# noahchalifour/rnnt-speech-recognition

Hardware: AMD Instinct MI355X
Metric: rnnt_loss_grad_lattice_cells_per_sec (higher is better)
Workload: dtype f32

## Files before the change

rnnt-speech-recognition_amd/csrc/rnnt_cell.h:

```cpp
#pragma once
#include "rnnt_common.h"

namespace rnnt {

__device__ __forceinline__ int length_T(const LossParams &p, const int b) { return min(max(p.input_lengths[b], 1), p.T); }
__device__ __forceinline__ int length_U(const LossParams &p, const int b) { return min(max(p.label_lengths[b] + 1, 1), p.U); }
__device__ __forceinline__ bool lengths_invalid(const LossParams &p, const int b) {
    const int t = p.input_lengths[b], l = p.label_lengths[b];
    return t < 1 || t > p.T || l < 0 || l > p.U - 1;
}

struct Cell {
    int b, t, u, Tb, Ub;
    bool valid;
};

__device__ __forceinline__ Cell decode(const LossParams &p, uint32_t c) {
    Cell r;
    r.b = r.t = r.u = r.Tb = r.Ub = 0;
    r.valid = false;
    if (c < p.cells) {
        const uint32_t row = fdiv(c, p.divU);
        r.u = (int)(c - row * (uint32_t)p.U);
        const uint32_t b = fdiv(row, p.divT);
        r.t = (int)(row - b * (uint32_t)p.T);
        r.b = (int)b;
        r.Tb = length_T(p, (int)b);
        r.Ub = length_U(p, (int)b);
        r.valid = (r.t < r.Tb) && (r.u < r.Ub);
    }
    return r;
}

__device__ __forceinline__ int clamp_label(int lab, int V) { return min(max(lab, 0), V - 1); }

template <bool SC1>
__device__ __forceinline__ float ld_f32(const float *q) {
    return SC1 ? __hip_atomic_load(q, __ATOMIC_RELAXED, __HIP_MEMORY_SCOPE_AGENT) : *q;
}
template <bool SC1>
__device__ __forceinline__ double ld_f64(const double *q) {
    return SC1 ? __hip_atomic_load(q, __ATOMIC_RELAXED, __HIP_MEMORY_SCOPE_AGENT) : *q;
}
__device__ __forceinline__ void st_f32_wt(float *q, float v) {
    __hip_atomic_store(q, v, __ATOMIC_RELAXED, __HIP_MEMORY_SCOPE_AGENT);
}
__device__ __forceinline__ void st_f64_wt(double *q, double v) {
    __hip_atomic_store(q, v, __ATOMIC_RELAXED, __HIP_MEMORY_SCOPE_AGENT);
}
struct CellGrad {
    float c0;
    float nl;
    float cb;
    float cl;
    bool has_blank_corr, has_label;
    int lab;
    float scale;
    float bscale, lscale;
};

template <bool SC1 = false>
__device__ __forceinline__ CellGrad cell_grad_from(const LossParams &p, const Cell &cl, uint32_t c, const float a, const float bt,
                                                   const float b_t1, const float b_u1) {
    CellGrad g;
    const int n = cl.t + cl.u;
    const int kc = n / kRebase, kc1 = (n + 1) / kRebase;
    const int g0 = (int)fdiv((uint32_t)cl.u, p.divOG), g1 = (int)fdiv((uint32_t)cl.u + 1u, p.divOG);
    const size_t ob = (size_t)cl.b * p.NC * p.NG;
    const double oa = (double)ld_f32<SC1>(p.offA + ob + (size_t)kc * p.NG + g0);
    const double ll2 = ld_f64<SC1>(p.ll + 2 * cl.b);
    const double da = (double)a + (oa - ll2);
    g.scale = p.cost_scale ? p.cost_scale[cl.b] : 1.0f;
    g.nl = -p.lse[c] * kLog2e;
    g.c0 = (float)(da + ((double)bt + (double)ld_f32<SC1>(p.offB + ob + (size_t)kc * p.NG + g0))) + g.nl;
    g.has_blank_corr = true;
    if (cl.t < cl.Tb - 1)
        g.cb = (float)(da + ((double)b_t1 + (double)ld_f32<SC1>(p.offB + ob + (size_t)kc1 * p.NG + g0)));
    else if (cl.u == cl.Ub - 1)
        g.cb = (float)da;
    else {
        g.cb = 0.f;
        g.has_blank_corr = false;
    }
    g.has_label = cl.u < cl.Ub - 1;
    g.lab = 0;
    g.cl = 0.f;
    if (g.has_label) {
        g.lab = clamp_label(p.labels[(size_t)cl.b * (p.U - 1) + cl.u], p.V);
        g.cl = (float)(da + ((double)b_u1 + (double)ld_f32<SC1>(p.offB + ob + (size_t)kc1 * p.NG + g1)));
    }
    return g;
}

__device__ __forceinline__ void fastemit_log(CellGrad &g, const float xl, const float lambda) {
    g.bscale = g.lscale = g.scale;
    if (g.has_label) {
        const float r = __builtin_amdgcn_exp2f(fminf((fmaf(xl, kLog2e, g.nl) + g.cl) - (g.c0 - g.nl), 0.f));
        g.lscale = fmaf(lambda, g.scale, g.scale);
        g.scale = fmaf(lambda * r, g.scale, g.scale);
    }
}

// ... 13 lines not shown
```

rnnt-speech-recognition_amd/csrc/rnnt_common.h:

```cpp
#pragma once
#include <hip/hip_runtime.h>
#include <stdint.h>

#include <type_traits>

namespace rnnt {

constexpr float kNeg = -1.0e30f;
constexpr float kNegTest = -1.0e29f;
constexpr float kLog2e = 1.4426950408889634f;
constexpr float kLn2 = 0.6931471805599453f;
constexpr int kRebase = 8;

struct FastDiv {
    uint32_t d, m, s;
};
inline FastDiv make_fastdiv(uint32_t d) {
    FastDiv f;
    f.d = d;
    uint32_t s = 0;
    while ((1ull << s) < d) ++s;
    f.s = s;
    f.m = (uint32_t)((((1ull << s) - d) << 32) / d) + 1u;
    return f;
}
__device__ __forceinline__ uint32_t fdiv(uint32_t n, const FastDiv f) {
    return (__umulhi(n, f.m) + n) >> f.s;
}

struct TileGeom {
    int TT, UU, tiles_t, tiles_u, cpr;
    FastDiv div_tu, div_tt, divUU, div_cpr, divTT;
};

struct LossParams {
    const float *acts;
    float *grads;
    const int *labels;
    const int *label_lengths;
    const int *input_lengths;
    const float *cost_scale;
    float *costs;
    float *lse;
    float *W;
    float *A;
    float *Bt;
    float *offA;
    float *offB;
    double *ll;
    int *EA;
    int *EB;
    float *lik;
    int *flags;
    int NCl;
    float2 *pstat;
    int *lshift;
    int *bar;
    int nPstat;
    int pstatStride;
    int B, T, U, V, blank;
    int b0, nb;
    int visit_all;
    int precise;
    int N, Nr, Up, NC, NG;
    uint32_t cells;
    FastDiv divU, divT, divV, divOG;
    TileGeom tile;
    float fe_lambda;
};

struct WsLayout {
    size_t lse, W, A, Bt, offA, offB, ll, EA, EB, lik, flags, pstat, lshift, bar, total;
    int NCl, nPstat;
    int N, Nr, Up, NC, NG, OG;
};

inline size_t align_up(size_t x, size_t a) { return (x + a - 1) / a * a; }

constexpr int kMaxU = 8192;
inline int sweep_K(int U) {
    const int k = (U + 63) / 64;
    const int avail[] = {1, 2, 3, 4, 6, 8, 12, 16};
    for (int a : avail)
        if (k <= a) return a;
    return 0;
}
template <int K, int G>
struct SweepRing {
    static constexpr size_t kChunk = (size_t)G * 2 * 64 * K * sizeof(float);
    static constexpr int NB = (4 * kChunk + 16 <= 128 * 1024) ? 4 : 3;
    static constexpr size_t kBytes = NB * kChunk + 16;
    static_assert(kBytes <= 160 * 1024, "chunk ring exceeds the LDS");
};
template <typename F>
inline hipError_t sweep_dispatch(int U, F &&f) {
    using std::integral_constant;
    switch (sweep_K(U)) {
        case 1: return f(integral_constant<int, 1>(), integral_constant<int, 16>());
        case 2: return f(integral_constant<int, 2>(), integral_constant<int, 16>());
        case 3: return f(integral_constant<int, 3>(), integral_constant<int, 16>());
        case 4: return f(integral_constant<int, 4>(), integral_constant<int, 16>());
        case 6: return f(integral_constant<int, 6>(), integral_constant<int, 8>());
        case 8: return f(integral_constant<int, 8>(), integral_constant<int, 8>());
        case 12: return f(integral_constant<int, 12>(), integral_constant<int, 4>());
        case 16: return f(integral_constant<int, 16>(), integral_constant<int, 4>());
        default: return hipErrorInvalidValue;
    }
}
constexpr int kFillByte = 0xF1;

inline WsLayout make_layout(int T, int U, int B) {
    WsLayout w;
    w.N = T + U - 1;
    w.Nr = (int)align_up((size_t)w.N, 16);
    w.Up = sweep_K(U) ? 64 * sweep_K(U) : (int)align_up((size_t)U, 64);
    w.NC = w.Nr / kRebase + 1;
    w.OG = sweep_K(U) ? sweep_K(U) : 64;
    w.NG = w.Up / w.OG;
    size_t off = 0;
    auto take = [&](size_t bytes) {
        size_t o = off;
        off = align_up(off + bytes, 256);
// ... 26 lines not shown
    TileGeom g;
    const int nu = (U + 31) / 32;
    g.UU = (U + nu - 1) / nu;
    g.TT = 256 / g.UU;
    if (g.TT > T) g.TT = T;
    g.tiles_u = (U + g.UU - 1) / g.UU;
    g.tiles_t = (T + g.TT - 1) / g.TT;
    g.cpr = g.UU * V / 4;
    g.div_tu = make_fastdiv((uint32_t)g.tiles_u);
    g.div_tt = make_fastdiv((uint32_t)g.tiles_t);
    g.divUU = make_fastdiv((uint32_t)g.UU);
    g.divTT = make_fastdiv((uint32_t)(g.TT > 0 ? g.TT : 1));
    g.div_cpr = make_fastdiv((uint32_t)(g.cpr > 0 ? g.cpr : 1));
    return g;
}

inline bool fill_loss_params(LossParams &p, const float *acts, float *grads, const int *labels, const int *label_lengths,
                             const int *input_lengths, const float *cost_scale, int V, int B, float *costs, void *workspace,
                             int maxT, int maxU, int blank) {
    const long long cells = (long long)B * maxT * maxU;
    if (cells <= 0 || cells >= (1ll << 31)) return false;
    if (((uintptr_t)workspace & 255) != 0) return false;
    const WsLayout w = make_layout(maxT, maxU, B);
    char *ws = (char *)workspace;
    p.acts = acts;
    p.grads = grads;
    p.labels = labels;
    p.label_lengths = label_lengths;
    p.input_lengths = input_lengths;
    p.cost_scale = cost_scale;
    p.costs = costs;
    p.lse = (float *)(ws + w.lse);
    p.W = (float *)(ws + w.W);
    p.A = (float *)(ws + w.A);
    p.Bt = (float *)(ws + w.Bt);
    p.offA = (float *)(ws + w.offA);
    p.offB = (float *)(ws + w.offB);
    p.ll = (double *)(ws + w.ll);
    p.EA = (int *)(ws + w.EA);
    p.EB = (int *)(ws + w.EB);
    p.lik = (float *)(ws + w.lik);
    p.flags = (int *)(ws + w.flags);
    p.NCl = w.NCl;
    p.pstat = (float2 *)(ws + w.pstat);
    p.lshift = (int *)(ws + w.lshift);
    p.bar = (int *)(ws + w.bar);
    p.nPstat = w.nPstat;
    p.pstatStride = 4;
    p.B = B, p.T = maxT, p.U = maxU, p.V = V, p.blank = blank;
    p.b0 = 0, p.nb = B;
    p.precise = 0;
    p.visit_all = 0;
    p.fe_lambda = 0.f;
    p.tile = make_tile(maxT, maxU, V);
    p.N = w.N, p.Nr = w.Nr, p.Up = w.Up, p.NC = w.NC, p.NG = w.NG;
    p.cells = (uint32_t)cells;
    p.divU = make_fastdiv((uint32_t)maxU);
    p.divT = make_fastdiv((uint32_t)maxT);
    p.divV = make_fastdiv((uint32_t)V);
    p.divOG = make_fastdiv((uint32_t)w.OG);
    return true;
}

constexpr float kExpTabLimit = 43.0f;
constexpr float kExpTab2Log2e = 2.8853900817779268f;
#ifdef __HIPCC__
__device__ __forceinline__ float exp_tab(float x) { return __builtin_amdgcn_exp2f(x * kExpTab2Log2e); }
__device__ __forceinline__ bool exp_tab_out_of_range(float x) { return !(fabsf(x) <= kExpTabLimit); }
#endif

constexpr int kHookBlocks = 1024;
struct JointHooks {
    int prep_mode;
    int prefilled;
    unsigned *dmax_enc;
    unsigned *dmax_pred;
};

#ifdef __HIPCC__
__device__ __forceinline__ void lds_dma16(const void *global, void *lds) {
    __builtin_amdgcn_global_load_lds((__attribute__((address_space(1))) const void *)global, (__attribute__((address_space(3))) void *)lds, 16, 0, 0);
}
#endif

inline int device_cu_count() {
    int dev = 0, n = 0;
    if (hipGetDevice(&dev) != hipSuccess) return 256;
    if (hipDeviceGetAttribute(&n, hipDeviceAttributeMultiprocessorCount, dev) != hipSuccess || n <= 0) return 256;
    return n;
}
template <typename Kernel>
inline hipError_t set_lds(Kernel kernel, size_t bytes) {
    if (bytes <= 64 * 1024) return hipSuccess;
    return hipFuncSetAttribute((const void *)kernel, hipFuncAttributeMaxDynamicSharedMemorySize, (int)bytes);
}

hipError_t launch_fill(void *dst, int byte, size_t bytes, hipStream_t s);
hipError_t launch_fill2(void *dst0, int byte0, size_t bytes0, void *dst1, int byte1, size_t bytes1, hipStream_t s);

bool tile_path_ok(const LossParams &p, bool grad);
hipError_t launch_lsm(const LossParams &p, hipStream_t s);
hipError_t launch_sweeps(const LossParams &p, hipStream_t s);
hipError_t launch_grad(const LossParams &p, hipStream_t s);
bool lin_path_ok(const LossParams &p);
hipError_t launch_lsm_lin(const LossParams &p, hipStream_t s);
hipError_t launch_sweeps_lin(const LossParams &p, hipStream_t s);
hipError_t launch_grad_lin(const LossParams &p, hipStream_t s);
hipError_t launch_redo_lin(const LossParams &p, bool force, hipStream_t s);

}
```

rnnt-speech-recognition_amd/csrc/rnnt_entrypoint.hip:

```cpp
#include "../../include/rnnt.h"
#include "rnnt_common.h"
#include "rnnt_lin.h"
#include "rnnt_align.h"
#include "rnnt_decode_host.h"

using namespace rnnt;

namespace rnnt {
hipError_t joint_workspace_bytes(int T, int U, int B, int J, int V, int joint_dtype, size_t *bytes);
hipError_t joint_f16_backward_rows(void *workspace, int T, int U, int B, int J, int V, int rows[2], hipStream_t s);
hipError_t joint_backward_rows(void *workspace, int T, int U, int B, int J, int V, int rows[2], hipStream_t s);
hipError_t launch_joint_loss(const float *enc_proj, const float *pred_proj, const float *W2, const float *b2,
                             const int *labels, const int *label_lengths, const int *input_lengths,
                             const float *cost_scale, int J, int V, int B, int T, int U, int blank, float *costs,
                             float *d_enc_proj, float *d_pred_proj, float *dW2, float *db2, int joint_dtype,
                             int phases, void *workspace, hipStream_t s, const JointHooks *hooks, float fe_lambda);
hipError_t joint_aux_pointers(void *workspace, int T, int U, int B, int J, int V, float **expE, float **expP, float **tflag);
hipError_t launch_joint_prefill(void *workspace, int T, int U, int B, int J, int V, hipStream_t s);
bool joint_dtype_supported(int joint_dtype, int J, int V);
bool dense_supported(int H, int J);
hipError_t dense_workspace_bytes(int B, int T, int U, int H, int J, size_t base, size_t *bytes);
void dense_proj_pointers(void *workspace, int B, int T, int U, int H, int J, size_t base, float **enc_proj, float **pred_proj,
                         float **d_enc_proj, float **d_pred_proj);
void dense_hook_pointers(void *workspace, int B, int T, int U, int H, int J, size_t base, unsigned **dmax_enc, unsigned **dmax_pred);
// ... 8 lines not shown
                                   int B, int T, int U, float *logits, void *workspace, hipStream_t s);
bool prednet_layout_ok(const rnntPrednetBlock *blocks, int L, int E, int V, int Jp, int R, size_t *bytes);
hipError_t launch_prednet_begin(const float *emb, const rnntPrednetBlock *blocks, int L, int E, int V, const float *W1, int Jp, int R,
                                float *out, void *workspace, hipStream_t s);
hipError_t launch_prednet_step(const int *emitted, const int *parents, float *out, const rnntPrednetBlock *blocks, int L, int E,
                               int V, int Jp, int R, void *workspace, hipStream_t s);
hipError_t launch_prednet_reset(const int *reset, float *out, const rnntPrednetBlock *blocks, int L, int E, int V, int Jp, int R,
                                void *workspace, hipStream_t s);
bool encoder_layout_ok(const rnntPrednetBlock *blocks, int L, int F, float bn_eps, int ridx, int f, int R, int Tmax, size_t *bytes);
hipError_t launch_encoder_begin(const rnntPrednetBlock *blocks, int L, int F, const float *bn_mean, const float *bn_var,
                                const float *bn_weight, const float *bn_bias, float bn_eps, int ridx, int f, int R, int Tmax,
                                void *workspace, hipStream_t s);
hipError_t launch_encoder_run(const float *x, int T, float *out, const rnntPrednetBlock *blocks, int L, int F, float bn_eps, int ridx,
                              int f, int R, int Tmax, void *workspace, hipStream_t s);
hipError_t launch_encoder_run_rows(const float *x, int T, const int *row_frames, const int *reset, float *out,
                                   const rnntPrednetBlock *blocks, int L, int F, float bn_eps, int ridx, int f, int R, int Tmax,
                                   void *workspace, hipStream_t s);
bool lstm_train_layout_ok(int R, int T, int H, int P, bool proj, size_t *bytes);
hipError_t launch_lstm_train_fwd(float *gates, const float *W_hh, const float *W_hr, float *y, float *c, float *h, int R, int T, int H,
                                 int P, void *workspace, hipStream_t s);
hipError_t launch_lstm_train_bwd(float *gates, const float *c, const float *dy, const float *W_hh, const float *W_hr, float *dr, int R,
                                 int T, int H, int P, void *workspace, hipStream_t s);
bool frontend_layout_ok(int K, int S, int L, int step, int M, int stack, int rm, size_t *bytes, int *max_rows);
hipError_t launch_frontend_begin(const float *window, const float *mel_weights, int K, int S, int L, int step, int M, int stack,
                                 int rm, void *workspace, hipStream_t s);
hipError_t launch_frontend_feed(const float *audio, int cs, const int *samples, const int *reset, const int *final_, int norm,
                                float *rows, int *counts, int K, int S, int L, int step, int M, int stack, int rm, void *workspace,
                                hipStream_t s);
}

extern "C" {

int get_warprnnt_version(void) { return 1; }

const char *rnntGetStatusString(rnntStatus_t status) {
    switch (status) {
        case RNNT_STATUS_SUCCESS: return "no error";
        case RNNT_STATUS_MEMOPS_FAILED: return "hip memcpy or memset failed";
        case RNNT_STATUS_INVALID_VALUE: return "invalid value";
        case RNNT_STATUS_EXECUTION_FAILED: return "execution failed";
        case RNNT_STATUS_UNKNOWN_ERROR:
        default: return "unknown error";
    }
}

rnntStatus_t get_workspace_size(int maxT, int maxU, int minibatch, bool gpu, size_t *size_bytes) {
    if (!size_bytes || maxT <= 0 || maxU <= 0 || minibatch <= 0 || !gpu) return RNNT_STATUS_INVALID_VALUE;
    *size_bytes = make_layout(maxT, maxU, minibatch).total;
    return RNNT_STATUS_SUCCESS;
}

static rnntStatus_t run_forward(LossParams &p, const WsLayout &w, hipStream_t s) {
    if (lin_path_ok(p)) {
        hipError_t e = launch_lsm_lin(p, s);
        if (e != hipSuccess) return from_hip(e);
        return from_hip(launch_sweeps_lin(p, s));
    }
    if (!tile_path_ok(p, false) && launch_fill(p.W, kFillByte, w.A - w.W, s) != hipSuccess) return RNNT_STATUS_MEMOPS_FAILED;
    p.precise = 1;
    hipError_t e = launch_lsm(p, s);
    if (e != hipSuccess) return from_hip(e);
    return from_hip(launch_sweeps(p, s));
}

static rnntStatus_t validate(const void *acts, const void *labels, const void *ll, const void *il, const void *ws,
                      int V, int B, const rnntOptions &o) {
    if (!acts || !labels || !ll || !il || !ws) return RNNT_STATUS_INVALID_VALUE;
    if (V <= 0 || B <= 0) return RNNT_STATUS_INVALID_VALUE;
    rnntStatus_t st = check_options(o);
    if (st != RNNT_STATUS_SUCCESS) return st;
    if (o.blank_label >= V) return RNNT_STATUS_INVALID_VALUE;
    return RNNT_STATUS_SUCCESS;
}

rnntStatus_t compute_rnnt_loss_fwd(const float *acts, const int *flat_labels, const int *label_lengths,
                                   const int *input_lengths, int alphabet_size, int minibatch, float *costs,
                                   void *workspace, rnntOptions options) {
    if (!costs) return RNNT_STATUS_INVALID_VALUE;
    rnntStatus_t st = validate(acts, flat_labels, label_lengths, input_lengths, workspace, alphabet_size, minibatch,
                               options);
    if (st != RNNT_STATUS_SUCCESS) return st;
    LossParams p;
    if (!fill_loss_params(p, acts, nullptr, flat_labels, label_lengths, input_lengths, nullptr, alphabet_size, minibatch, costs,
                          workspace, options.maxT, options.maxU, options.blank_label))
        return RNNT_STATUS_INVALID_VALUE;
    hipStream_t s = (hipStream_t)options.stream;
    const WsLayout w = make_layout(options.maxT, options.maxU, minibatch);
    st = run_forward(p, w, s);
    if (st != RNNT_STATUS_SUCCESS || !lin_path_ok(p)) return st;
    return from_hip(launch_redo_lin(p, false, s));
}

static rnntStatus_t run_backward(LossParams &p, hipStream_t s) {
    if (!lin_path_ok(p)) return from_hip(launch_grad(p, s));
    const bool patch = tile_path_ok(p, true);
    if (patch) {
        hipError_t e = launch_grad_lin(p, s);
        if (e != hipSuccess) return from_hip(e);
    }
    return from_hip(launch_redo_lin(p, !patch, s));
}

rnntStatus_t compute_rnnt_loss_bwd(const float *acts, float *grads, const int *flat_labels,
                                   const int *label_lengths, const int *input_lengths, const float *cost_scale,
                                   int alphabet_size, int minibatch, void *workspace, rnntOptions options) {
    if (!grads) return RNNT_STATUS_INVALID_VALUE;
// ... 901 lines not shown
```

rnnt-speech-recognition_amd/csrc/rnnt_kernels.hip:

```cpp
#include "rnnt_common.h"
#include "rnnt_cell.h"
#include "rnnt_sweep.h"
#include "rnnt_cellwave.h"
#include "rnnt_lin.h"
#include "rnnt_cellbody.h"

#include <float.h>
#include <math.h>
#include <stdlib.h>

namespace rnnt {


typedef float gs_v4f __attribute__((ext_vector_type(4)));
__device__ __forceinline__ void grad_store16(gs_v4f *dst, const gs_v4f v) { __builtin_nontemporal_store(v, dst); }

constexpr int kFillRows = 16;

template <int VP, bool GRAD, bool AL = true, bool LIN = false, bool FE = false>
__global__ __launch_bounds__(256) void cell_tile_kernel(const LossParams p) {
    extern __shared__ __attribute__((aligned(16))) float lds[];
    const int tid = threadIdx.x;
    const int lane = tid & 63;
    const int wave = __builtin_amdgcn_readfirstlane(tid >> 6);
    const int V = p.V;
    const TileGeom &tg = p.tile;
    const uint32_t n_patch_wg = (uint32_t)p.nb * (uint32_t)tg.tiles_t * (uint32_t)tg.tiles_u;
    uint32_t vblock = blockIdx.x;
    if (!GRAD) {
        const uint32_t per = (uint32_t)p.Nr / kFillRows, n_fill = (uint32_t)p.nb * per;
        const uint32_t pgs = (n_patch_wg + 7u) >> 3, fgs = (n_fill + 7u) >> 3, P = (pgs + fgs) / fgs;
        const uint32_t g = blockIdx.x >> 3, l8 = blockIdx.x & 7u;
        const uint32_t k = g / P;
        const bool is_fill = g - k * P == P - 1u && k < fgs;
        if (is_fill) {
            const uint32_t f = k * 8u + l8;
            if (f >= n_fill) return;
            const int fb = p.b0 + (int)(f / per), chunk = (int)(f % per);
            const int Tf = length_T(p, fb), Uf = length_U(p, fb);
            const int Nf = Tf + Uf - 1;
            float2 *Wb = (float2 *)p.W + (size_t)fb * p.Nr * p.Up;
            const float2 z = LIN ? make_float2(0.f, 0.f) : make_float2(kNeg, kNeg);
            for (int idx = tid; idx < kFillRows * p.Up; idx += 256) {
                const int rr = idx / p.Up, u = idx - rr * p.Up;
                const int n = chunk * kFillRows + rr;
                if (n < Nf && (u < max(0, n - Tf + 1) || u > min(n, Uf - 1))) Wb[(size_t)n * p.Up + u] = z;
            }
            return;
        }
        vblock = (g - min(k, fgs)) * 8u + l8;
        if (vblock >= n_patch_wg) return;
    }
    uint32_t bid;
    {
        const uint32_t nwg = n_patch_wg, xcd = vblock & 7u, idx = vblock >> 3;
        const uint32_t q = nwg >> 3, r = nwg & 7u;
        bid = (xcd < r ? xcd * (q + 1u) : r * (q + 1u) + (xcd - r) * q) + idx;
        if (GRAD) bid = (xcd < r ? xcd * (q + 1u) : r * (q + 1u) + (xcd - r) * q) + ((xcd < r ? q + 1u : q) - 1u - idx);
    }
    const uint32_t q1 = fdiv(bid, tg.div_tu);
    const uint32_t tu = bid - q1 * (uint32_t)tg.tiles_u;
    const uint32_t bb = fdiv(q1, tg.div_tt);
    const uint32_t tt = q1 - bb * (uint32_t)tg.tiles_t;
    const int b = p.b0 + (int)bb;
    const int t0 = (int)tt * tg.TT, u0 = (int)tu * tg.UU;
    int len_t = p.input_lengths[b], len_l = p.label_lengths[b];
    LinUtt ut = {};
    if (GRAD && LIN) {
        int4 fl = lin_flag_words(p, b);
        ut.sh = p.lshift[b];
        ut.mL = p.lik[4 * b];
        ut.EL = ((const int *)p.lik)[4 * b + 1];
        float sc = *(p.cost_scale ? p.cost_scale + b : p.lik + 4 * b);
        asm volatile("" : "+s"(len_t), "+s"(len_l), "+s"(fl.x), "+s"(fl.y), "+s"(fl.w), "+s"(ut.sh), "+s"(ut.mL), "+s"(ut.EL), "+s"(sc));
        ut.scale = p.cost_scale ? sc : 1.0f;
        if (lin_skip_words(fl)) return;
    } else {
        asm volatile("" : "+s"(len_t), "+s"(len_l));
    }
    const int Tb = min(max(len_t, 1), p.T), Ub = min(max(len_l + 1, 1), p.U);

    const int rows_valid = max(0, min(tg.TT, Tb - t0));
    const int cols_valid = max(0, min(tg.UU, Ub - u0));
    const int rows_in = max(0, min(tg.TT, p.T - t0));
    const int cols_in = max(0, min(tg.UU, p.U - u0));
    const int q_valid = cols_valid * V / 4;
    const int q_in = cols_in * V / 4;
    const int row_lds = AL ? tg.UU * V : ((tg.UU * V + 3 + 3) & ~3);
    const size_t row_f = (size_t)p.U * V;
    const size_t patch0 = ((size_t)(b * p.T + t0) * p.U + u0) * V;

    auto store_row = [&](const int r, const float *src) {
        const size_t s0 = patch0 + r * row_f;
        if (AL) {
            for (int q = lane; q < q_in; q += 64) {
                typedef float v4f __attribute__((ext_vector_type(4)));
                const v4f v = src ? ((const v4f *)src)[q] : (v4f){0.f, 0.f, 0.f, 0.f};
                grad_store16((v4f *)(p.grads + s0 + q * 4), v);
            }
        } else {
            const int a = (int)(s0 & 3), len = cols_in * V;
            float *base = p.grads + (s0 - a);
            for (int q = lane; q * 4 < a + len; q += 64) {
                const int e0 = q * 4 - a;
                typedef float v4f __attribute__((ext_vector_type(4)));
                const v4f vv = src ? ((const v4f *)src)[q] : (v4f){0.f, 0.f, 0.f, 0.f};
                const float v[4] = {vv[0], vv[1], vv[2], vv[3]};
                if (e0 >= 0 && e0 + 3 < len) {
                    grad_store16((v4f *)(base + q * 4), vv);
                } else {
#pragma unroll
                    for (int k = 0; k < 4; ++k)
                        if (e0 + k >= 0 && e0 + k < len) base[q * 4 + k] = v[k];
                }
            }
        }
    };

    float2 *const pslot = p.pstat + (size_t)b * p.nPstat + ((size_t)tt * tg.tiles_u + tu) * 4 + wave;
    if (rows_valid == 0 || cols_valid == 0) {
        if (GRAD) {
            for (int r = wave; r < rows_in; r += 4) store_row(r, nullptr);
        }
        if (!GRAD && LIN && wave == 0 && lane == 0) *pslot = make_float2(0.f, 0.f);
        return;
    }

    const uint32_t r = fdiv((uint32_t)tid, tg.divUU);
    const int cu = tid - (int)r * tg.UU;
    Cell cl;
    cl.b = b, cl.t = t0 + (int)r, cl.u = u0 + cu, cl.Tb = Tb, cl.Ub = Ub;
    cl.valid = ((int)r < rows_valid) && (cu < cols_valid);
    const uint32_t c = ((uint32_t)(b * p.T + cl.t)) * (uint32_t)p.U + (uint32_t)cl.u;

    LinGrad lg = {};
    if (!GRAD && cl.valid && cl.u < Ub - 1) lg.lab = p.labels[(size_t)b * (p.U - 1) + cl.u];
    uint32_t lword = ~0u;
    if (GRAD && LIN) {
        bool live = false;
        if (cl.valid) {
            lg = lin_grad_setup(p, cl, ut);
            if (lg.bad) atomicOr(p.flags + 4 * cl.b + kFlagG, 1);
            live = p.visit_all || !(lg.l2occ <= (float)-kOccFloorWave);
            cl.valid = live;
        }
        const uint64_t m = __ballot(live);
        const int ncell = tg.TT * tg.UU, nw = (ncell + 31) >> 5;
        uint32_t *const lw = (uint32_t *)lds;
        if (lane == 0 && wave * 64 < ncell) lw[2 * wave] = (uint32_t)m;
        if (lane == 0 && wave * 64 + 32 < ncell) lw[2 * wave + 1] = (uint32_t)(m >> 32);
        __syncthreads();
        lword = lane < nw ? lw[lane] : 0u;
        __syncthreads();
        if (__ballot(lword != 0u) == 0) {
            for (int rr = wave; rr < rows_in; rr += 4) store_row(rr, nullptr);
            return;
        }
    }
    auto cells_live = [&](const int klo, const int khi) -> bool {
        const uint32_t wlo = (uint32_t)__shfl((int)lword, klo >> 5), whi = (uint32_t)__shfl((int)lword, khi >> 5);
        const uint64_t bits = ((uint64_t)whi << 32 | wlo) >> (klo & 31);
        return (bits & ((2ull << (khi - klo)) - 1ull)) != 0;
    };

    for (int r = wave; r < rows_valid; r += 4) {
        const size_t s0 = patch0 + r * row_f;
        const int a = AL ? 0 : (int)(s0 & 3);
        const float *src = p.acts + (s0 - a);
        float *dst = lds + r * row_lds;
        const int nq = AL ? q_valid : (a + cols_valid * V + 3) / 4;
        for (int q0 = 0; q0 < nq; q0 += 64) {
            const int q = q0 + lane;
            bool need = q < nq;
            if (GRAD && LIN) {
                const int e = min(q, nq - 1) * 4 - a;
                const int lo = (int)fdiv((uint32_t)max(0, e), p.divV), hi = AL ? lo : (int)fdiv((uint32_t)min(e + 3, cols_valid * V - 1), p.divV);
                need = cells_live(r * tg.UU + lo, r * tg.UU + hi) && need;
            }
            if (need) {
                __builtin_amdgcn_global_load_lds((glb_void *)(src + q * 4), (lds_void *)(dst + q0 * 4), 16, 0, 0);
            }
        }
    }
    wait_vm0();
    __syncthreads();
    if (!GRAD) asm volatile("" : "+v"(lg.lab));

    float stat = 0.f;
    if (AL) {
        if ((GRAD && tid < tg.TT * tg.UU) || cl.valid) stat = cell_body<VP, true, GRAD, LIN, false, FE>(p, cl, c, lds + tid * V, lds + tid * V, &lg);
    } else if ((int)r < tg.TT) {
        const int a = (int)((patch0 + r * row_f) & 3);
        if (GRAD || cl.valid) stat = cell_body<VP, false, GRAD, LIN, false, FE>(p, cl, c, lds + r * row_lds + a + cu * V, lds + r * row_lds + a + cu * V, &lg);
    }
    if (!GRAD && LIN) {
        if (wave == 0) {
            const float cnt = (float)__popcll(__ballot(cl.valid));
            stat = cl.valid ? stat : 0.f;
            stat += __int_as_float(__builtin_amdgcn_update_dpp(0, __float_as_int(stat), 0xB1 , 0xf, 0xf, true));
            stat += __int_as_float(__builtin_amdgcn_update_dpp(0, __float_as_int(stat), 0x4E , 0xf, 0xf, true));
            stat += __int_as_float(__builtin_amdgcn_update_dpp(0, __float_as_int(stat), 0x141 , 0xf, 0xf, true));
            stat += __int_as_float(__builtin_amdgcn_update_dpp(0, __float_as_int(stat), 0x140 , 0xf, 0xf, true));
            const float sum = (__builtin_amdgcn_readlane(stat, 0) + __builtin_amdgcn_readlane(stat, 16)) +
                              (__builtin_amdgcn_readlane(stat, 32) + __builtin_amdgcn_readlane(stat, 48));
            if (lane == 0) *pslot = make_float2(sum, cnt);
        }
        __syncthreads();
        float2 *const Wp = (float2 *)p.W + ((size_t)b * p.Nr + t0 + u0) * p.Up + u0;
// ... 294 lines not shown
```

rnnt-speech-recognition_amd/csrc/rnnt_lin.h:

```cpp
#pragma once
#include "rnnt_sweep.h"

namespace rnnt {

__host__ __device__ constexpr int lin_shift_max(int K) { return (K == 1 || K >= 12) ? 2 : 3; }
constexpr float kLinDecayBits = 6.2f;
constexpr int kLinDrag = 118;
constexpr int kFrameNone = -(1 << 28);
constexpr int kCertBits = -40;
constexpr float kTinyEdge = 7.8886091e-31f;

enum { kFlagA = 0, kFlagB = 1, kFlagG = 2, kFlagState = 3 };

__device__ __forceinline__ void st_i32_wt(int *q, int v) { __hip_atomic_store(q, v, __ATOMIC_RELAXED, __HIP_MEMORY_SCOPE_AGENT); }
__device__ __forceinline__ float frexp_m(float x) { return __builtin_amdgcn_frexp_mantf(x); }
__device__ __forceinline__ int frexp_e(float x) { return __builtin_amdgcn_frexp_expf(x); }
__device__ __forceinline__ float ldexp_f(float x, int e) { return __builtin_ldexpf(x, e); }

__device__ __forceinline__ bool lin_skip_words(const int4 fl) { return (fl.x | fl.y) != 0 || fl.w == 2; }
__device__ __forceinline__ int4 lin_flag_words(const LossParams &p, const int b) { return *(const int4 *)(p.flags + 4 * b); }
__device__ __forceinline__ bool lin_skip(const LossParams &p, const int b) { return lin_skip_words(lin_flag_words(p, b)); }

struct LinUtt {
    int sh;
    float mL;
    int EL;
    float scale;
};

struct LinIdx {
    size_t sk;
    size_t down;
    size_t diag;
    size_t e00, e10, e11;
    size_t lab;
};
__host__ __device__ __forceinline__ LinIdx lin_grad_indices(const int b, const int n, const int u, const int sh, const int l0, const int l1,
                                                            const int Nr, const int Up, const int NCl, const int U) {
    LinIdx x;
    const int n1 = n + 1 < Nr ? n + 1 : Nr - 1, u1 = u + 1 < Up ? u + 1 : Up - 1;
    x.sk = ((size_t)b * Nr + n) * Up + u;
    x.down = ((size_t)b * Nr + n1) * Up + u;
    x.diag = ((size_t)b * Nr + n1) * Up + u1;
    const int kc = n >> sh, kc1 = (n + 1) >> sh;
    const int kcc = kc < NCl ? kc : NCl - 1, kc1c = kc1 < NCl ? kc1 : NCl - 1;
    const int l1c = l1 < 64 ? l1 : 63;
    const size_t tb = (size_t)b * NCl * 64;
    x.e00 = tb + (size_t)kcc * 64 + l0;
    x.e10 = tb + (size_t)kc1c * 64 + l0;
    x.e11 = tb + (size_t)kc1c * 64 + l1c;
    const int ul = u < U - 2 ? u : U - 2;
    x.lab = (size_t)b * (U - 1) + (ul > 0 ? ul : 0);
    return x;
}

template <int VP>
__device__ __forceinline__ float lin_cell_lsm(const LossParams &p, const Cell &cl, const float (&x)[VP], const float *xs, const int lab) {
    float m = x[0];
#pragma unroll
    for (int i = 1; i < VP; ++i) m = fmaxf(m, x[i]);
    float s = 0.f;
    const float nml = -m * kLog2e;
#pragma unroll
    for (int i = 0; i < VP; ++i) s += ex2(fmaf(x[i], kLog2e, nml));
    const float inv = __builtin_amdgcn_rcpf(s);
    const bool blank_stays = (cl.t < cl.Tb - 1) || (cl.u == cl.Ub - 1);
    float pb = 0.f, pl = 0.f;
    if (blank_stays) {
        pb = ex2(fmaf(xs[p.blank], kLog2e, nml)) * inv;
        if (!(pb >= kTinyEdge)) pb = NAN;
    }
    if (cl.u < cl.Ub - 1) {
        pl = ex2(fmaf(xs[lab], kLog2e, nml)) * inv;
        if (!(pl >= kTinyEdge)) pl = NAN;
    }
    float *const xo = const_cast<float *>(xs);
    xo[0] = pb, xo[1] = pl;
    const float best = fmaxf(pb, pl);
    return (pb != pb || pl != pl) ? 200.f : -lg2(fmaxf(best, 1.0e-37f));
}

struct LinGrad {
    float h0;
    float hb;
    float hl;
    float l2occ;
    bool has_blank_corr, has_label, bad;
    int lab;
};

__device__ __forceinline__ LinGrad lin_grad_setup(const LossParams &p, const Cell &cl, const LinUtt &ut) {
    LinGrad g;
    const int n = cl.t + cl.u;
    const int l0 = (int)fdiv((uint32_t)cl.u, p.divOG), l1 = (int)fdiv((uint32_t)cl.u + 1u, p.divOG);
    const LinIdx ix = lin_grad_indices(cl.b, n, cl.u, ut.sh, l0, l1, p.Nr, p.Up, p.NCl, p.U);
    const float ma = p.A[ix.sk], mb = p.Bt[ix.sk];
    const float m_dn = p.Bt[ix.down], m_dg = p.Bt[ix.diag];
    const int ea = p.EA[ix.e00], eb = p.EB[ix.e00];
    const int e_dn = p.EB[ix.e10], e_dg = p.EB[ix.e11];
    const int labw = *(p.U > 1 ? p.labels + ix.lab : (const int *)p.lshift + cl.b);
    const bool down = cl.t < cl.Tb - 1;
    g.has_label = cl.u < cl.Ub - 1;
    const float mL = ut.mL;
    const int EL = ut.EL;
    const float scale = ut.scale;
    const int xa = frexp_e(ma), xb = frexp_e(mb);
    const float qa = scale * frexp_m(ma) * __builtin_amdgcn_rcpf(mL);
// ... 27 lines not shown
```

rnnt-speech-recognition_amd/csrc/rnnt_lin_kernels.hip:

```cpp
#include "rnnt_common.h"
#include "rnnt_cell.h"
#include "rnnt_sweep.h"
#include "rnnt_cellwave.h"
#include "rnnt_lin.h"
#include "rnnt_cellbody.h"
#include "rnnt_redo.h"

namespace rnnt {

__device__ __forceinline__ float dpp_lower_zero(float x) {
    return __int_as_float(__builtin_amdgcn_update_dpp(0, __float_as_int(x), 0x138 , 0xf, 0xf, true));
}
__device__ __forceinline__ float dpp_upper_zero(float x) {
    return __int_as_float(__builtin_amdgcn_update_dpp(0, __float_as_int(x), 0x130 , 0xf, 0xf, true));
}
__device__ __forceinline__ int dpp_lower_i(int x, int fill) {
    return __builtin_amdgcn_update_dpp(fill, x, 0x138, 0xf, 0xf, false);
}
__device__ __forceinline__ int dpp_upper_i(int x, int fill) {
    return __builtin_amdgcn_update_dpp(fill, x, 0x130, 0xf, 0xf, false);
}

struct LinState {
    int E;
    int d;
    int *tab;
    float *row;
};

template <int K, bool BETA, int SH>
__device__ __forceinline__ void lin_renorm(float (&v)[K], LinState &st, const int kc) {
    float m = v[0];
#pragma unroll
    for (int j = 1; j < K; ++j) m = fmaxf(m, v[j]);
    const int own = (m > 0.f) ? st.E + frexp_e(m) : kFrameNone;
    constexpr int LOOK = ((1 << SH) + K - 1) / K;
    int nb = own, reach = kFrameNone;
#pragma unroll
    for (int r = 0; r < LOOK; ++r) {
        nb = BETA ? dpp_upper_i(nb, kFrameNone) : dpp_lower_i(nb, kFrameNone);
        reach = max(reach, nb);
    }
    const int En = max(own, reach - kLinDrag);
    const int sh = st.E - En;
#pragma unroll
    for (int j = 0; j < K; ++j) v[j] = ldexp_f(v[j], sh);
    st.E = En;
    const int up = dpp_upper_i(En, En);
    st.d = BETA ? up - En : En - up;
    st_i32_wt(st.tab + (size_t)kc * 64, En);
}

template <int K>
struct LinRow {
    static constexpr bool WIDE = (K % 2) == 0;
    static constexpr int NR = WIDE ? K / 2 : K;
    f32x4 q4[WIDE ? K / 2 : 1];
    f32x2 q2[WIDE ? 1 : K];
    template <int J>
// ... 233 lines not shown
    const int Tb = length_T(p, b), Ub = length_U(p, b);
    const int Nb = Tb + Ub - 1;
    float *out = p.Bt + (size_t)b * p.Nr * Up;
    const int voff = lane * K * 4;
    const int u0 = lane * K;

    float bv[K];
#pragma unroll
    for (int j = 0; j < K; ++j) bv[j] = (u0 + j == Ub - 1) ? 1.f : 0.f;
    const int last = Nb - 1;
    const int ckl = last / G;
    LinState st;
    st.E = 0, st.d = 0;
    st.tab = p.EB + (size_t)b * p.NCl * 64 + lane;
    st.row = out + (size_t)last * Up;

    LandedView lv;
    lv.addr0 = lk.landed;
#pragma unroll
    for (int w = 0; w < kLinLoaders; ++w) lv.have[w] = 0;
    bool timed_out = lengths_invalid(p, b);
    for (int ck = ckl; ck >= 0; --ck) {
        const int i_ring = ckl - ck;
        timed_out |= !lv.wait(i_ring);
        const float *cur = bufs + (i_ring % NB) * chunkf + 2 * u0;
        const int r0 = ck * G;
        if (r0 + G - 1 < last) {
            const uint32_t abase = (uint32_t)(uintptr_t)((lds_void *)cur);
            LinRow<K> wq[3];
            lin_issue_row<K, G - 1>(wq[0], abase);
            lin_issue_row<K, G - 2>(wq[1], abase);
            lin_beta_fast_steps<K, G, SH, 0>(bv, wq, abase, st, voff, lane, r0);
        } else {
            for (int ii = 0; ii < G; ++ii) {
                const int i = G - 1 - ii;
                const int n = r0 + i;
                if (n > last) continue;
                LinRow<K> wc;
                lin_load_row<K>(wc, cur + i * 2 * Up);
                lin_beta_step<K>(bv, wc, st.d);
                if ((n & ((1 << SH) - 1)) == (1 << SH) - 1 || n == last) lin_renorm<K, true, SH>(bv, st, n >> SH);
                store_diag<K, false>(st.row, voff, lane, bv);
                st.row -= Up;
            }
        }
        if (ck > 0) {
            asm volatile("s_waitcnt lgkmcnt(0)" ::: "memory");
            if (lane == 0) lds_post(lk.consumed, i_ring + 1);
        }
    }
    if (lane == 0) lin_record(p, b, 1, bv[0], st.E, timed_out);
}

template <int K, int G, int NB>
__global__ __launch_bounds__(64 * (1 + kLinLoaders)) void lin_sweep_kernel(const LossParams p) {
    extern __shared__ __attribute__((aligned(16))) float lds[];
    constexpr int chunkf = G * 2 * 64 * K;
    const int tid = threadIdx.x, lane = tid & 63;
    const int wave = __builtin_amdgcn_readfirstlane(tid >> 6);
    const int b = p.b0 + (int)(blockIdx.x >> 1);
    const bool beta = (blockIdx.x & 1) != 0;
    int *ctr = (int *)(lds + NB * chunkf);
    if (tid < 2 * kLinLoaders) ctr[tid] = 0;
    __syncthreads();
    LdLink lk;
    lk.landed = (uint32_t)(uintptr_t)((lds_void *)ctr);
    lk.consumed = lk.landed + 4u;
    if (wave >= 1) {
        LdLink mine = lk;
        mine.landed = lk.landed + 8u * (uint32_t)(wave - 1);
        if (beta)
            sweep_loader<K, G, NB, true, kLinLoaders>(p, lds, mine, b, lane, wave - 1);
        else
            sweep_loader<K, G, NB, false, kLinLoaders>(p, lds, mine, b, lane, wave - 1);
    } else {
        constexpr int SHmax = lin_shift_max(K);
        int sh = SHmax;
        if constexpr (SHmax > 2) {
            float sum = 0.f, cnt = 0.f;
            const float2 *ps = p.pstat + (size_t)b * p.nPstat;
            const int stride = p.pstatStride, npatch = p.nPstat / stride;
            for (int i0 = 0; i0 < npatch; i0 += 512) {
                float2 q[8];
#pragma unroll
                for (int k = 0; k < 8; ++k) {
                    const int i = i0 + 64 * k + lane;
                    q[k] = (i < npatch) ? ps[(size_t)stride * i] : make_float2(0.f, 0.f);
                }
#pragma unroll
                for (int k = 0; k < 8; ++k) sum += q[k].x, cnt += q[k].y;
            }
#pragma unroll
            for (int off = 32; off > 0; off >>= 1) sum += __shfl_xor(sum, off), cnt += __shfl_xor(cnt, off);
            sh = (sum > kLinDecayBits * cnt) ? 2 : SHmax;
            sh = __builtin_amdgcn_readfirstlane(sh);
        }
        if constexpr (SHmax > 2) {
            if (sh == 2) {
                if (beta)
                    lin_beta_sweep<K, G, NB, 2>(p, lds, lk, b, lane);
                else
                    lin_alpha_sweep<K, G, NB, 2>(p, lds, lk, b, lane);
                return;
            }
        }
        if (beta)
            lin_beta_sweep<K, G, NB, SHmax>(p, lds, lk, b, lane);
        else
            lin_alpha_sweep<K, G, NB, SHmax>(p, lds, lk, b, lane);
    }
}

template <int K, int G, int NB, bool FE = false>
__global__ __launch_bounds__(kRedoThreads) void lin_redo_kernel(const LossParams p, const int force, const int team) {
    extern __shared__ __attribute__((aligned(16))) float lds[];
    constexpr int chunkf = G * 2 * 64 * K;
    const int tid = threadIdx.x;
    const int ub = (int)blockIdx.x / team;
    const int b = p.b0 + ub;
    RedoTeam tm;
    tm.k = (int)blockIdx.x - ub * team, tm.n = team, tm.bar = p.bar + kRedoCtr * b, tm.ok = true;
    int *fl = p.flags + 4 * b;
    typedef int i32x4 __attribute__((ext_vector_type(4)));
    typedef double f64x2 __attribute__((ext_vector_type(2)));
    const i32x4 fw = __builtin_nontemporal_load((const i32x4 *)fl);
    const f64x2 lw = __builtin_nontemporal_load((const f64x2 *)(p.ll + 2 * b));
    const int state = fw[kFlagState];
    bool redo = false;
    if (state != 2) {
        const bool agree = fabs(lw[0] - lw[1]) * 0.6931471805599453 <= 2e-5 + 1e-8 * fabs(lw[0]);
        redo = force || (fw[kFlagA] | fw[kFlagB] | fw[kFlagG]) != 0 || !agree;
        if (!redo) return;
    } else if (!p.grads) {
        return;
    }
    if (redo) redo_lattice<K, G, NB>(p, b, tm, lds, tid);
    uint32_t lo, hi;
    redo_cell_range(p, b, tm, lo, hi);
    if (p.grads) redo_cells<true, FE>(p, lo, hi, tid, lds, NB * chunkf);
    if (!tm.ok) {
        if (p.costs && tm.k == 0 && tid == 0) st_f32_wt(p.costs + b, NAN);
        if (p.grads)
            for (size_t i = (size_t)lo * p.V + tid; i < (size_t)hi * p.V; i += kRedoThreads) p.grads[i] = NAN;
    }
}

bool lin_path_ok(const LossParams &p) { return p.V >= 2 && sweep_K(p.U) >= 1 && tile_path_ok(p, false); }

template <int K, int G>
static hipError_t launch_lin_sweep(const LossParams &p, hipStream_t s) {
    using R = SweepRing<K, G>;
    static_assert(2 * kLinLoaders * sizeof(int) <= 16, "the loaders' flag words exceed the ring's 16 bytes");
    hipError_t e = set_lds(lin_sweep_kernel<K, G, R::NB>, R::kBytes);
    if (e != hipSuccess) return e;
    hipLaunchKernelGGL((lin_sweep_kernel<K, G, R::NB>), dim3(2 * p.nb), dim3(64 * (1 + kLinLoaders)), R::kBytes, s, p);
    return hipGetLastError();
}
template <int K, int G, bool FE = false>
static hipError_t launch_lin_redo(const LossParams &p, const bool force, hipStream_t s) {
    using R = SweepRing<K, G>;
    hipError_t e = set_lds(lin_redo_kernel<K, G, R::NB, FE>, R::kBytes);
    if (e != hipSuccess) return e;
    const int team = redo_team_size(p.nb, p.T, p.U, device_cu_count());
    hipLaunchKernelGGL((lin_redo_kernel<K, G, R::NB, FE>), dim3(p.nb * team), dim3(kRedoThreads), R::kBytes, s, p, force ? 1 : 0, team);
    return hipGetLastError();
}

hipError_t launch_sweeps_lin(const LossParams &p, hipStream_t s) {
    return sweep_dispatch(p.U, [&](auto K, auto G) { return launch_lin_sweep<K, G>(p, s); });
}
hipError_t launch_redo_lin(const LossParams &p, const bool force, hipStream_t s) {
    if (p.grads && p.fe_lambda != 0.f)
        return sweep_dispatch(p.U, [&](auto K, auto G) { return launch_lin_redo<K, G, true>(p, force, s); });
    return sweep_dispatch(p.U, [&](auto K, auto G) { return launch_lin_redo<K, G>(p, force, s); });
}

}
```

Measured before the change: 14.53 billion.

## Zero out-of-range gradient patches in idle helper blocks during the sweep kernel

Adds extra helper blocks to the alpha/beta sweep launch that use otherwise idle CUs to write zeros into gradient tiles lying outside each sequence's valid lattice. The later gradient kernel then skips those tiles. This moves zero-fill traffic off the critical gradient pass and overlaps it with the latency-bound sweep. An env-controlled 'far' threshold for skipping tiles far from the diagonal exists but is off by default. The cost is extra memory traffic competing with the sweep, plus a dependence on free CU count.

```diff
diff --git a/rnnt-speech-recognition_amd/csrc/rnnt_cell.h b/rnnt-speech-recognition_amd/csrc/rnnt_cell.h
--- a/rnnt-speech-recognition_amd/csrc/rnnt_cell.h
+++ b/rnnt-speech-recognition_amd/csrc/rnnt_cell.h
@@ -48,6 +48,39 @@
 __device__ __forceinline__ void st_f64_wt(double *q, double v) {
     __hip_atomic_store(q, v, __ATOMIC_RELAXED, __HIP_MEMORY_SCOPE_AGENT);
 }
+typedef float gs_v4f __attribute__((ext_vector_type(4)));
+__device__ __forceinline__ void grad_store16(gs_v4f *dst, const gs_v4f v) { __builtin_nontemporal_store(v, dst); }
+
+template <bool AL>
+__device__ __forceinline__ void patch_store_row(float *grads, const size_t s0, const int len, const float *src, const int lane) {
+    if (AL) {
+        for (int q = lane; q < len / 4; q += 64) {
+            const gs_v4f v = src ? ((const gs_v4f *)src)[q] : (gs_v4f){0.f, 0.f, 0.f, 0.f};
+            grad_store16((gs_v4f *)(grads + s0 + q * 4), v);
+        }
+    } else {
+        const int a = (int)(s0 & 3);
+        float *base = grads + (s0 - a);
+        for (int q = lane; q * 4 < a + len; q += 64) {
+            const int e0 = q * 4 - a;
+            const gs_v4f vv = src ? ((const gs_v4f *)src)[q] : (gs_v4f){0.f, 0.f, 0.f, 0.f};
+            const float v[4] = {vv[0], vv[1], vv[2], vv[3]};
+            if (e0 >= 0 && e0 + 3 < len) {
+                grad_store16((gs_v4f *)(base + q * 4), vv);
+            } else {
+#pragma unroll
+                for (int k = 0; k < 4; ++k)
+                    if (e0 + k >= 0 && e0 + k < len) base[q * 4 + k] = v[k];
+            }
+        }
+    }
+}
+template <bool AL>
+__device__ __forceinline__ void patch_zero_rows(float *grads, const size_t patch0, const size_t row_f, const int rows_in, const int len,
+                                                const int wave, const int nw, const int lane) {
+    for (int r = wave; r < rows_in; r += nw) patch_store_row<AL>(grads, patch0 + r * row_f, len, nullptr, lane);
+}
+
 struct CellGrad {
     float c0;
     float nl;
diff --git a/rnnt-speech-recognition_amd/csrc/rnnt_common.h b/rnnt-speech-recognition_amd/csrc/rnnt_common.h
--- a/rnnt-speech-recognition_amd/csrc/rnnt_common.h
+++ b/rnnt-speech-recognition_amd/csrc/rnnt_common.h
@@ -67,7 +67,10 @@
     FastDiv divU, divT, divV, divOG;
     TileGeom tile;
     float fe_lambda;
-};
+    int far;
+    int prezeroed;
+};
+constexpr int kPrezeroFarOff = -1;
 
 struct WsLayout {
     size_t lse, W, A, Bt, offA, offB, ll, EA, EB, lik, flags, pstat, lshift, bar, total;
@@ -200,7 +203,8 @@
     p.precise = 0;
     p.visit_all = 0;
     p.fe_lambda = 0.f;
-    p.tile = make_tile(maxT, maxU, V);
+    p.far = kPrezeroFarOff, p.prezeroed = 0;
+    p.tile =make_tile(maxT, maxU, V);
     p.N = w.N, p.Nr = w.Nr, p.Up = w.Up, p.NC = w.NC, p.NG = w.NG;
     p.cells = (uint32_t)cells;
     p.divU = make_fastdiv((uint32_t)maxU);
@@ -255,5 +259,7 @@
 hipError_t launch_sweeps_lin(const LossParams &p, hipStream_t s);
 hipError_t launch_grad_lin(const LossParams &p, hipStream_t s);
 hipError_t launch_redo_lin(const LossParams &p, bool force, hipStream_t s);
-
-}
+int prezero_helpers(const LossParams &p);
+int prezero_far_setting();
+
+}
diff --git a/rnnt-speech-recognition_amd/csrc/rnnt_entrypoint.hip b/rnnt-speech-recognition_amd/csrc/rnnt_entrypoint.hip
--- a/rnnt-speech-recognition_amd/csrc/rnnt_entrypoint.hip
+++ b/rnnt-speech-recognition_amd/csrc/rnnt_entrypoint.hip
@@ -84,6 +84,8 @@
 
 static rnntStatus_t run_forward(LossParams &p, const WsLayout &w, hipStream_t s) {
     if (lin_path_ok(p)) {
+        p.prezeroed = prezero_helpers(p);
+        if (p.prezeroed) p.far = prezero_far_setting();
         hipError_t e = launch_lsm_lin(p, s);
         if (e != hipSuccess) return from_hip(e);
         return from_hip(launch_sweeps_lin(p, s));
diff --git a/rnnt-speech-recognition_amd/csrc/rnnt_kernels.hip b/rnnt-speech-recognition_amd/csrc/rnnt_kernels.hip
--- a/rnnt-speech-recognition_amd/csrc/rnnt_kernels.hip
+++ b/rnnt-speech-recognition_amd/csrc/rnnt_kernels.hip
@@ -11,9 +11,6 @@
 
 namespace rnnt {
 
-
-typedef float gs_v4f __attribute__((ext_vector_type(4)));
-__device__ __forceinline__ void grad_store16(gs_v4f *dst, const gs_v4f v) { __builtin_nontemporal_store(v, dst); }
 
 constexpr int kFillRows = 16;
 
@@ -90,37 +87,15 @@
     const size_t row_f = (size_t)p.U * V;
     const size_t patch0 = ((size_t)(b * p.T + t0) * p.U + u0) * V;
 
-    auto store_row = [&](const int r, const float *src) {
-        const size_t s0 = patch0 + r * row_f;
-        if (AL) {
-            for (int q = lane; q < q_in; q += 64) {
-                typedef float v4f __attribute__((ext_vector_type(4)));
-                const v4f v = src ? ((const v4f *)src)[q] : (v4f){0.f, 0.f, 0.f, 0.f};
-                grad_store16((v4f *)(p.grads + s0 + q * 4), v);
-            }
-        } else {
-            const int a = (int)(s0 & 3), len = cols_in * V;
-            float *base = p.grads + (s0 - a);
-            for (int q = lane; q * 4 < a + len; q += 64) {
-                const int e0 = q * 4 - a;
-                typedef float v4f __attribute__((ext_vector_type(4)));
-                const v4f vv = src ? ((const v4f *)src)[q] : (v4f){0.f, 0.f, 0.f, 0.f};
-                const float v[4] = {vv[0], vv[1], vv[2], vv[3]};
-                if (e0 >= 0 && e0 + 3 < len) {
-                    grad_store16((v4f *)(base + q * 4), vv);
-                } else {
-#pragma unroll
-                    for (int k = 0; k < 4; ++k)
-                        if (e0 + k >= 0 && e0 + k < len) base[q * 4 + k] = v[k];
-                }
-            }
-        }
+    auto store_row = [&](const int r, const float *src) { patch_store_row<AL>(p.grads, patch0 + r * row_f, cols_in * V, src, lane); };
+    auto prezeroed = [&]() -> bool {
+        return GRAD && LIN && p.prezeroed && prezero_patch(tg, Tb, Ub, (int)tt, (int)tu, prezero_far(p));
     };
 
     float2 *const pslot = p.pstat + (size_t)b * p.nPstat + ((size_t)tt * tg.tiles_u + tu) * 4 + wave;
     if (rows_valid == 0 || cols_valid == 0) {
-        if (GRAD) {
-            for (int r = wave; r < rows_in; r += 4) store_row(r, nullptr);
+        if (GRAD && !prezeroed()) {
+            patch_zero_rows<AL>(p.grads, patch0, row_f, rows_in, cols_in * V, wave, 4, lane);
         }
         if (!GRAD && LIN && wave == 0 && lane == 0) *pslot = make_float2(0.f, 0.f);
         return;
@@ -153,7 +128,7 @@
         lword = lane < nw ? lw[lane] : 0u;
         __syncthreads();
         if (__ballot(lword != 0u) == 0) {
-            for (int rr = wave; rr < rows_in; rr += 4) store_row(rr, nullptr);
+            if (!prezeroed()) patch_zero_rows<AL>(p.grads, patch0, row_f, rows_in, cols_in * V, wave, 4, lane);
             return;
         }
     }
diff --git a/rnnt-speech-recognition_amd/csrc/rnnt_lin.h b/rnnt-speech-recognition_amd/csrc/rnnt_lin.h
--- a/rnnt-speech-recognition_amd/csrc/rnnt_lin.h
+++ b/rnnt-speech-recognition_amd/csrc/rnnt_lin.h
@@ -53,6 +53,18 @@
     x.lab = (size_t)b * (U - 1) + (ul > 0 ? ul : 0);
     return x;
 }
+
+__host__ __device__ __forceinline__ bool prezero_far_point(const long long t2, const long long u2, const int Tb, const int Ub, const int far) {
+    const long long d = u2 * Tb - t2 * Ub;
+    return (d < 0 ? -d : d) * 512 > (long long)far * Tb * Ub;
+}
+__host__ __device__ __forceinline__ bool prezero_patch(const TileGeom &tg, const int Tb, const int Ub, const int tt, const int tu, const int far) {
+    const int t0 = tt * tg.TT, u0 = tu * tg.UU;
+    if (t0 >= Tb || u0 >= Ub) return true;
+    if (far < 0) return false;
+    return prezero_far_point(2ll * t0 + tg.TT, 2ll * u0 + tg.UU, Tb, Ub, far);
+}
+__host__ __device__ __forceinline__ int prezero_far(const LossParams &p) { return p.visit_all ? kPrezeroFarOff : p.far; }
 
 template <int VP>
 __device__ __forceinline__ float lin_cell_lsm(const LossParams &p, const Cell &cl, const float (&x)[VP], const float *xs, const int lab) {
diff --git a/rnnt-speech-recognition_amd/csrc/rnnt_lin_kernels.hip b/rnnt-speech-recognition_amd/csrc/rnnt_lin_kernels.hip
--- a/rnnt-speech-recognition_amd/csrc/rnnt_lin_kernels.hip
+++ b/rnnt-speech-recognition_amd/csrc/rnnt_lin_kernels.hip
@@ -5,6 +5,8 @@
 #include "rnnt_lin.h"
 #include "rnnt_cellbody.h"
 #include "rnnt_redo.h"
+
+#include <stdlib.h>
 
 namespace rnnt {
 
@@ -344,12 +346,45 @@
     if (lane == 0) lin_record(p, b, 1, bv[0], st.E, timed_out);
 }
 
+constexpr int kPrezeroHelpers = 192;
+constexpr int kPrezeroFar = kPrezeroFarOff;
+
+template <bool AL>
+__device__ __forceinline__ void prezero_helper(const LossParams &p, const uint32_t h, const uint32_t H, const int wave, const int lane) {
+    const TileGeom &tg = p.tile;
+    const uint32_t nrows = (uint32_t)p.nb * (uint32_t)tg.tiles_t;
+    const int far = prezero_far(p);
+    const size_t row_f = (size_t)p.U * p.V;
+    for (uint32_t q = h; q < nrows; q += H) {
+        const uint32_t bb = fdiv(q, tg.div_tt);
+        const int tt = (int)(q - bb * (uint32_t)tg.tiles_t), b = p.b0 + (int)bb;
+        const int Tb = length_T(p, b), Ub = length_U(p, b);
+        const int t0 = tt * tg.TT;
+        const int rows_in = max(0, min(tg.TT, p.T - t0));
+        for (int tu = 0; tu < tg.tiles_u; ++tu) {
+            if (!prezero_patch(tg, Tb, Ub, tt, tu, far)) continue;
+            const int u0 = tu * tg.UU;
+            const int cols_in = max(0, min(tg.UU, p.U - u0));
+            const size_t patch0 = ((size_t)(b * p.T + t0) * p.U + u0) * p.V;
+            patch_zero_rows<AL>(p.grads, patch0, row_f, rows_in, cols_in * p.V, wave, 1 + kLinLoaders, lane);
+        }
+    }
+}
+
 template <int K, int G, int NB>
 __global__ __launch_bounds__(64 * (1 + kLinLoaders)) void lin_sweep_kernel(const LossParams p) {
     extern __shared__ __attribute__((aligned(16))) float lds[];
     constexpr int chunkf = G * 2 * 64 * K;
     const int tid = threadIdx.x, lane = tid & 63;
     const int wave = __builtin_amdgcn_readfirstlane(tid >> 6);
+    if (blockIdx.x >= 2u * (uint32_t)p.nb) {
+        const uint32_t h = blockIdx.x - 2u * (uint32_t)p.nb, H = gridDim.x - 2u * (uint32_t)p.nb;
+        if ((p.V % 4) == 0)
+            prezero_helper<true>(p, h, H, wave, lane);
+        else
+            prezero_helper<false>(p, h, H, wave, lane);
+        return;
+    }
     const int b = p.b0 + (int)(blockIdx.x >> 1);
     const bool beta = (blockIdx.x & 1) != 0;
     int *ctr = (int *)(lds + NB * chunkf);
@@ -445,8 +480,21 @@
     static_assert(2 * kLinLoaders * sizeof(int) <= 16, "the loaders' flag words exceed the ring's 16 bytes");
     hipError_t e = set_lds(lin_sweep_kernel<K, G, R::NB>, R::kBytes);
     if (e != hipSuccess) return e;
-    hipLaunchKernelGGL((lin_sweep_kernel<K, G, R::NB>), dim3(2 * p.nb), dim3(64 * (1 + kLinLoaders)), R::kBytes, s, p);
+    hipLaunchKernelGGL((lin_sweep_kernel<K, G, R::NB>), dim3(2 * p.nb + p.prezeroed), dim3(64 * (1 + kLinLoaders)), R::kBytes, s, p);
     return hipGetLastError();
+}
+
+int prezero_helpers(const LossParams &p) {
+    if (kPrezeroHelpers <= 0 || !p.grads || !lin_path_ok(p) || !tile_path_ok(p, true)) return 0;
+    const int free_cus = device_cu_count() - 2 * p.nb;
+    if (2 * free_cus < kPrezeroHelpers) return 0;
+    return free_cus < kPrezeroHelpers ? free_cus : kPrezeroHelpers;
+}
+int prezero_far_setting() {
+    const char *e = getenv("RNNT_PREZERO_FAR");
+    if (!e || !*e) return kPrezeroFar;
+    const long v = strtol(e, nullptr, 10);
+    return v < 0 ? kPrezeroFarOff : (v > 4096 ? 4096 : (int)v);
 }
 template <int K, int G, bool FE = false>
 static hipError_t launch_lin_redo(const LossParams &p, const bool force, hipStream_t s) {
```

Result: no change. 14.67 billion, median of 4 (+1.0%).
